# jermp/sshash

Hardware: AMD Instinct MI355X
Metric: k-mer Lookups/sec (batched random queries, bit-exact ids) (higher is better)
Workload: dtype u64

## Files before the change

### sshash_amd/csrc/engine.hip

```cpp
#include <hip/hip_runtime.h>

#include <algorithm>
#include <atomic>
#include <cstdlib>
#include <cstring>
#include <mutex>
#include <exception>
#include <stdexcept>
#include <thread>

#include "engine.hpp"
#include "hooks.hpp"
#include "replica.hpp"
#include "sktable.hpp"

namespace sshash_amd {

static void check_single_launch(uint64_t lanes, char const* what) {
    if (lanes >= (uint64_t(1) << 32))
        throw error(error_kind::argument, std::string(what) + ": at most 2^32 - 1 lanes per call (split the batch)");
}


int visible_device_count() {
// ... 103 lines not shown
        for (uint32_t b = a + 1; b < count;) {
            if (((e[a] >> 40) & 0xFFFF) == ((e[b] >> 40) & 0xFFFF)) {
                e[b] = e[count - 1];
                e[count - 1] = 0;
                --count;
                overflow = true;
            } else {
                ++b;
            }
        }
    }
    if (overflow) e[0] |= uint64_t(1) << 63;
    for (uint32_t j = 0; j < DIR_SLOTS; ++j) B[j] = e[j];
    if (overflow) atomicAdd(stats, 1ull);
    atomicAdd(stats + 1, (unsigned long long)count);
}

engine::engine(std::shared_ptr<host_index> idx) : m_idx(std::move(idx)) {}
engine::~engine() = default;

bool engine::on_device(int device) const {
    std::shared_lock<std::shared_mutex> lock(m_replicas_mutex);
    for (auto const& r : m_replicas)
        if (r->device == device) return true;
    return false;
}

std::vector<int> engine::devices() const {
    std::vector<int> d;
    std::shared_lock<std::shared_mutex> lock(m_replicas_mutex);
    for (auto const& r : m_replicas) d.push_back(r->device);
    return d;
}

uint64_t engine::device_bytes(int device) const { return replica(device)->bytes; }

void engine::device_stats(int device, uint64_t out[16]) const {
    device_replica const* r = replica(device);
    out[0] = r->bytes;
    out[1] = r->view.directory.enabled ? r->view.directory.num_buckets : 0;
    out[2] = r->directory_overflowed;
    out[3] = r->directory_entries;
    out[4] = r->view.sk.enabled ? uint64_t(r->view.sk.num_buckets) * SK_BUCKET_SLOTS +
                                      uint64_t(r->view.sk.kmer_buckets) * (r->view.k > 31 ? SK_BUCKET_SLOTS : SK_KMER_ENTRIES_NARROW)
                                : 0;
    out[5] = r->sk_keys;
    out[6] = r->sk_keys - r->sk_heavy_keys;
    out[7] = r->sk_unplaced;
    out[8] = r->sk_slots_used;
    out[9] = r->sk_heavy_keys;
    out[10] = r->sk_heavy_kmers;
    out[11] = r->view.sk.enabled ? 0 : r->sk_absent_reason;
    out[12] = r->sk_bytes;
    out[13] = r->view.sk.m;
    out[14] = out[15] = 0;
}

void engine::device_table_histogram(int device, uint64_t out[32]) const {
    device_replica const* r = replica(device);
    for (int i = 0; i < 32; ++i) out[i] = i < 20 && r->view.sk.enabled ? r->sk_histogram[i] : 0;
}

device_replica const* engine::replica(int device) const {
    std::shared_lock<std::shared_mutex> lock(m_replicas_mutex);
    for (auto const& r : m_replicas)
        if (r->device == device) return r.get();
    throw error(error_kind::no_device, "dictionary is not resident on device " + std::to_string(device) +
                             " (call sshash_to_device first)");
}

char const* isa_guard_state() {
#if defined(SSHASH_ISA_GUARDED)
    return "guarded";
#else
    return "plain";
#endif
}

void engine::to_device(int device, uint32_t table_shards, uint32_t table_shard_id) {
#if !defined(SSHASH_ISA_GUARDED)
    {
        static std::once_flag once;
        std::call_once(once, [] {
            fprintf(stderr, "[sshash_amd] WARNING: this library was NOT built through tools/isa_guard.py (make -C sshash_amd/csrc): on gfx950 a "
                                "kernel that keeps a 64-bit shift amount in the last VGPR of its allocation computes wrongly some of the time "
                                "(HISTORY.md); tests/test_isa_guard.py names the kernels of a build that are exposed\n");
        });
    }
#endif
    if (table_shards == 0 || table_shard_id >= table_shards) throw error(error_kind::argument, "table shard id must be < number of table shards");
    std::lock_guard<std::mutex> one_upload_at_a_time(m_upload_mutex);
    {
        std::shared_lock<std::shared_mutex> lock(m_replicas_mutex);
        for (auto const& r : m_replicas) {
            if (r->device != device) continue;
            if (r->view.sk.num_shards != table_shards || r->view.sk.shard_id != table_shard_id)
                throw error(error_kind::argument, "the dictionary is already resident on device " + std::to_string(device) +
                                                      " with another table sharding (" + std::to_string(r->view.sk.shard_id) + " of " +
                                                      std::to_string(r->view.sk.num_shards) + ")");
            return;
        }
    }
    const int count = visible_device_count();
    if (count == 0) throw error(error_kind::no_device, "no HIP device visible: the lookup path requires an MI355X (no CPU fallback)");
    if (device < 0 || device >= count) throw error(error_kind::no_device, "invalid device ordinal " + std::to_string(device));
    device_guard guard(device);
    host_index const& idx = *m_idx;
    auto rep = std::make_unique<device_replica>();
    rep->device = device;
    dict_view& v = rep->view;
    v.k = idx.k;
    v.m = idx.m;
    v.canonical = idx.canonical;
    v.skew_parts = idx.skew_num_partitions;
    v.hash_magic = idx.hash_magic;
    v.num_kmers = idx.num_kmers;
    v.num_strings = idx.num_strings;
    v.num_bases = idx.num_bases;
    {
        const uint32_t nt = std::max(1u, std::min(16u, std::thread::hardware_concurrency()));
        std::vector<granule> g = make_granules(idx, nt);
        if (idx.k <= 31) {
            std::vector<atom32> a = make_atoms(g, nt);
            std::vector<granule>().swap(g);
            v.granules = rep->put(a);
        } else {
            v.granules = rep->put(g);
        }
    }
    v.endpoints = rep->put(idx.endpoints);
    v.minimizers = rep->put_mphf(idx.minimizers_mphf);
    v.cw_width = idx.control_codewords.width;
    v.off_width = idx.mid_load_buckets.width;
    v.begin_buckets_of_size = rep->put(idx.begin_buckets_of_size);
    v.mid_load = rep->put(idx.mid_load_buckets.words);
    v.heavy_load = rep->put(idx.heavy_load_buckets.words);
    v.heavy_size = idx.heavy_load_buckets.size;
    v.codewords = nullptr;
    v.cw_packed = 0;
    v.directory.buckets = nullptr;
    v.directory.num_buckets = 0;
    v.directory.enabled = 0;
    rep->bytes_still_to_come = 8 * sizeof(skew_part_dev);
    for (uint32_t p = 0; p < 8; ++p) {
        if (p < idx.skew_num_partitions && idx.skew_mphfs[p].num_keys) {
            mphf_host const& f = idx.skew_mphfs[p];
            rep->bytes_still_to_come += f.parts.size() * sizeof(f.parts[0]) + (f.pilots.size() + f.free_slots.size() + idx.skew_positions[p].words.size()) * 8;
        } else {
            rep->bytes_still_to_come += 64;
        }
    }
    if (idx.weighted()) rep->bytes_still_to_come += (idx.weight_starts.size() + idx.weight_values.size()) * 8;
    build_sk_table(*rep, idx, table_shards, table_shard_id);
    const char* dir_env = std::getenv("SSHASH_AMD_DIRECTORY");
    const bool lean = v.sk.enabled && !(dir_env && dir_env[0] == '1');
    if (lean) {
        v.codewords = rep->put(idx.control_codewords.words);
        v.cw_packed = 1;
    } else {
        const uint64_t n = idx.control_codewords.size;
        device_buffers tmp;
        uint64_t* packed = tmp.alloc<uint64_t>(idx.control_codewords.words.size());
        HIP_CHECK(hipMemcpy(packed, idx.control_codewords.words.data(), idx.control_codewords.words.size() * sizeof(uint64_t), hipMemcpyHostToDevice));
        uint64_t* wide = tmp.alloc<uint64_t>(std::max<uint64_t>(n, 1));
        tmp.keep(wide, *rep);
        rep->bytes += std::max<uint64_t>(n, 1) * sizeof(uint64_t);
        if (n) {
            check_single_launch(n, "upload (one lane per minimizer)");
            hipLaunchKernelGGL(widen_codewords_kernel, dim3(uint32_t((n + 255) / 256)), dim3(256), 0, 0, v, packed, n, wide);
            HIP_CHECK(hipGetLastError());
            HIP_CHECK(hipDeviceSynchronize());
        }
        v.codewords = wide;
    }
    if (!lean) {
        const bool want = !(dir_env && dir_env[0] == '0');
        const uint64_t n = idx.control_codewords.size;
        const uint64_t nb = uint64_t(double(n) / DIR_LOAD) + 1;
        if (want && n && nb < (uint64_t(1) << 32) && v.cw_width <= DIR_CODE_BITS) {
            device_buffers tmp;
            uint64_t* buckets = tmp.alloc<uint64_t>(nb * 4);
            uint32_t* claimed = tmp.alloc<uint32_t>(nb);
            unsigned long long* stats = tmp.alloc<unsigned long long>(2);
            HIP_CHECK(hipMemset(buckets, 0, nb * 32));
            HIP_CHECK(hipMemset(claimed, 0, nb * 4));
            HIP_CHECK(hipMemset(stats, 0, 16));
            tmp.keep(buckets, *rep);
            rep->bytes += nb * 32;
            hipLaunchKernelGGL(directory_insert_kernel, dim3(uint32_t((n + 255) / 256)), dim3(256), 0, 0, v, n, buckets, claimed, uint32_t(nb));
            hipLaunchKernelGGL(directory_finalize_kernel, dim3(uint32_t((nb + 255) / 256)), dim3(256), 0, 0, buckets, claimed, uint32_t(nb), stats);
            HIP_CHECK(hipGetLastError());
            unsigned long long h_stats[2];
            HIP_CHECK(hipMemcpy(h_stats, stats, 16, hipMemcpyDeviceToHost));
            rep->directory_overflowed = h_stats[0];
            rep->directory_entries = h_stats[1];
            v.directory.buckets = buckets;
            v.directory.num_buckets = uint32_t(nb);
            v.directory.enabled = 1;
        }
    }
    std::vector<skew_part_dev> skew(8);
    for (uint32_t p = 0; p < 8; ++p) {
        std::memset(&skew[p], 0, sizeof(skew_part_dev));
        if (p < idx.skew_num_partitions && idx.skew_mphfs[p].num_keys) {
            skew[p].f = rep->put_mphf(idx.skew_mphfs[p]);
            skew[p].positions = rep->put(idx.skew_positions[p].words);
            skew[p].pos_width = idx.skew_positions[p].width;
        } else {
            mphf_host dummy;
            dummy.pilot_width = 1;
            dummy.num_keys = 1;
            mphf_partition part{};
            part.num_keys = 1;
            part.table_size = 1;
            part.dense_buckets = 1;
            part.sparse_buckets = 1;
            dummy.parts.push_back(part);
            dummy.pilots.assign(2, 0);
            dummy.free_slots.assign(1, 0);
            skew[p].f = rep->put_mphf(dummy);
            skew[p].positions = rep->put(std::vector<uint64_t>(2, 0));
            skew[p].pos_width = 1;
        }
    }
    rep->d_skew = rep->put(skew);
    v.weight_starts = v.weight_values = nullptr;
    v.num_weight_intervals = idx.weight_values.size();
    if (idx.weighted()) {
        v.weight_starts = rep->put(idx.weight_starts);
        v.weight_values = rep->put(idx.weight_values);
    }
    rep->create_scratch_pool();
    if (const uint64_t budget = hbm_budget(); budget && rep->bytes > budget)
        throw error(error_kind::no_device, "the replica needs " + std::to_string(rep->bytes) + " bytes of HBM, SSHASH_AMD_HBM_BUDGET allows " +
                                               std::to_string(budget) + ": partition the dictionary (minimizer shards, table shards)");
    std::unique_lock<std::shared_mutex> lock(m_replicas_mutex);
    m_replicas.push_back(std::move(rep));
}


template <int W, bool CANON, int MODE, bool ASCII>
__global__ void __launch_bounds__(256)
lookup_kernel(const dict_view d, const skew_part_dev* __restrict__ skew, const void* __restrict__ queries,
              const uint64_t n, const bool check_rc, const result_view out, uint8_t* __restrict__ member,
              const uint8_t* __restrict__ lane_valid) {
    const uint64_t stride = uint64_t(gridDim.x) * blockDim.x;
    for (uint64_t i = uint64_t(blockIdx.x) * blockDim.x + threadIdx.x; i < n; i += stride) {
        if (lane_valid && !(lane_valid[i] & 1)) continue;
        kmer_w<W> x;
        if constexpr (ASCII) {
            x = kmer_from_ascii<W>(static_cast<const char*>(queries) + i * d.k, d.k);
        } else {
            const uint64_t* q = static_cast<const uint64_t*>(queries) + i * W;
            for (int j = 0; j < W; ++j) x.w[j] = q[j];
            x = kmer_take_chars<W>(x, d.k);
        }
        const hit_t h = lookup_one<W, CANON, MODE != int(out_mode::full)>(d, skew, x, check_rc);
        if constexpr (MODE == int(out_mode::member)) {
            member[i] = h.found ? 1 : 0;
        } else {
            store_result<MODE == int(out_mode::full)>(d, out, i, h);
        }
    }
}

constexpr uint32_t DEFER_SHARDS = 2048;
constexpr uint32_t DEFER_BLOCKS_PER_SHARD = 4;

struct pass_queues {
    uint32_t* defer_counts;
    uint32_t* resume_counts;
    uint32_t* defer_index;
    uint32_t* resume_index;
    uint64_t* resume_kmers;
    uint64_t* resume_meta;
    uint32_t defer_capacity;
    uint32_t resume_capacity;
    uint32_t flag_misses;
};
constexpr uint32_t DEFER_FLAG_ONLY = 1u << 31;

template <int W, bool ASCII>
__device__ __forceinline__ kmer_w<W> load_query(const void* __restrict__ queries, uint64_t i, uint32_t k) {
    kmer_w<W> x;
    if constexpr (ASCII) {
        x = kmer_from_ascii<W>(static_cast<const char*>(queries) + i * k, k);
    } else {
        const uint64_t* q = static_cast<const uint64_t*>(queries) + i * W;
        for (int j = 0; j < W; ++j) x.w[j] = __builtin_nontemporal_load(q + j);
        x = kmer_take_chars<W>(x, k);
    }
    return x;
}

template <int W, bool CANON, int MODE, bool ASCII, bool SK>
__global__ void __launch_bounds__(256, (W == 2 && SK) ? 8 : 1)
fast_lookup_kernel(const dict_view d, const void* __restrict__ queries, const uint64_t n, const bool check_rc,
                   const result_view out, uint8_t* __restrict__ member, const pass_queues q,
                   const uint8_t* __restrict__ lane_valid ) {
    constexpr uint32_t TILE_WORDS = ASCII ? 64 * (W == 1 ? 31 : 63) + 24 : 0;
    constexpr uint32_t STAGE_WORDS = SK ? 256 * 16 : 0;
    __shared__ uint4 lds[(TILE_WORDS > STAGE_WORDS ? TILE_WORDS : STAGE_WORDS) / 4 + 1];
    const uint64_t i = uint64_t(blockIdx.x) * blockDim.x + threadIdx.x;
    const bool active = i < n && (!lane_valid || (lane_valid[i] & 1));
    kmer_w<W> x = kmer_zero<W>();
    if constexpr (ASCII) {
        uint32_t* tile = reinterpret_cast<uint32_t*>(lds);
        const uint64_t first = uint64_t(blockIdx.x) * blockDim.x;
        const uint32_t count = uint32_t(n - first < blockDim.x ? n - first : blockDim.x);
        const uint32_t bytes = count * d.k;
        const char* src = static_cast<const char*>(queries) + first * d.k;
        if ((reinterpret_cast<uintptr_t>(src) & 15) == 0) {
            for (uint32_t c = threadIdx.x; c * 16 < bytes; c += blockDim.x) {
                if (c * 16 + 16 <= bytes) {
                    reinterpret_cast<uint4*>(tile)[c] = sk_load_piece(src + 16 * c);
                } else {
                    for (uint32_t b = c * 16; b < bytes; ++b) reinterpret_cast<char*>(tile)[b] = src[b];
                }
            }
        } else {
            for (uint32_t b = threadIdx.x; b < bytes; b += blockDim.x) reinterpret_cast<char*>(tile)[b] = src[b];
        }
        __syncthreads();
        if (active) {
            const uint32_t start = threadIdx.x * d.k, w0 = start >> 2, sh = start & 3;
            uint32_t acc[2 * W];
#pragma unroll
            for (int t = 0; t < 2 * W; ++t) {
                acc[t] = 0;
                if (16u * uint32_t(t) < d.k) {
                    uint32_t prev = tile[w0 + 4 * t];
#pragma unroll
                    for (int j = 0; j < 4; ++j) {
                        const uint32_t next = tile[w0 + 4 * t + j + 1];
                        const uint32_t four = __builtin_amdgcn_alignbyte(next, prev, sh);
                        prev = next;
                        const uint32_t c = (((four >> 1) & 0x03030303u) * 0x01041040u) >> 24;
                        acc[t] |= c << (8 * j);
                    }
                }
            }
            x.w[0] = uint64_t(acc[0]) | (uint64_t(acc[1]) << 32);
            if constexpr (W == 2) x.w[1] = uint64_t(acc[2]) | (uint64_t(acc[3]) << 32);
            x = kmer_take_chars<W>(x, d.k);
        }
        if constexpr (SK) __syncthreads();
    } else {
        if (active) x = load_query<W, false>(queries, i, d.k);
    }
    fast_t r;
    const uint32_t shard = blockIdx.x & (DEFER_SHARDS - 1);
    if constexpr (SK) {
        if constexpr (W == 1)
            r = sk_lookup_in_wave<W>(d, x, active, CANON || check_rc, (!CANON && check_rc) ? int8_t(-1) : int8_t(1), lds + (threadIdx.x >> 6) * (64 * 4));
        else
            r = sk_first_pass_wave<W>(d, x, active, CANON || check_rc, (!CANON && check_rc) ? int8_t(-1) : int8_t(1),
                                      lds + (threadIdx.x >> 6) * (64 * 4));
        bool resume = active && r.outcome == FAST_CONTINUE;
        const uint32_t place = wave_queue_place(resume, q.resume_counts + shard);
        if (resume) {
            if (place < q.resume_capacity) {
                const uint64_t at = uint64_t(shard) * q.resume_capacity + place;
                q.resume_index[at] = uint32_t(i) | uint32_t(r.kmer_offset);
                for (int j = 0; j < W; ++j) q.resume_kmers[at * W + j] = x.w[j];
            } else {
                r.outcome = FAST_DEFER;
            }
        }
        if (!active) return;
    } else {
        bool by_pairs = false;
        if constexpr (W == 1 && !CANON) by_pairs = (d.num_bases >> 37) == 0;
        if (by_pairs) {
            if constexpr (W == 1 && !CANON) r = fast_lookup_pairs(d, x, active, check_rc);
        } else {
            r = active ? fast_lookup_one<W, CANON>(d, x, check_rc) : fast_unsettled(false);
        }
        const bool scan = active && r.outcome == FAST_SCAN;
        const uint32_t place = wave_queue_place(scan, q.resume_counts + shard);
        if (scan) {
            if (place < q.resume_capacity) {
                const uint64_t at = uint64_t(shard) * q.resume_capacity + place;
                q.resume_index[at] = uint32_t(i);
                q.resume_meta[at] = r.kmer_offset;
                for (int j = 0; j < W; ++j) q.resume_kmers[at * W + j] = x.w[j];
            } else {
                r.outcome = FAST_DEFER;
            }
        }
        if (!active) return;
    }
    if constexpr (MODE == int(out_mode::member)) {
        __builtin_nontemporal_store(uint8_t(r.outcome == FAST_HIT ? 1 : 0), member + i);
    } else {
        hit_t h;
        h.kmer_offset = r.kmer_offset;
        h.string_id = r.string_id;
        h.orientation = r.orientation;
        h.found = r.outcome == FAST_HIT;
        h.minimizer_found = true;
        store_result<MODE == int(out_mode::full)>(d, out, i, h);
    }
    if (r.outcome == FAST_DEFER) q.defer_index[uint64_t(shard) * q.defer_capacity + atomicAdd(q.defer_counts + shard, 1u)] = uint32_t(i);
    else if (MODE == int(out_mode::full) && SK && q.flag_misses && r.outcome == FAST_MISS)
        q.defer_index[uint64_t(shard) * q.defer_capacity + atomicAdd(q.defer_counts + shard, 1u)] = uint32_t(i) | DEFER_FLAG_ONLY;
}

constexpr uint32_t RESUME_PARTS = 4;

template <int W, bool CANON, int MODE>
__global__ void __launch_bounds__(256)
resume_lookup_kernel(const dict_view d, const bool check_rc, const result_view out, uint8_t* __restrict__ member, const pass_queues q) {
    __shared__ uint4 lds[256 * 4];
    const uint32_t shard = blockIdx.x & (DEFER_SHARDS - 1), part = blockIdx.x / DEFER_SHARDS;
    const uint32_t pushed = q.resume_counts[shard];
    const uint32_t total = pushed < q.resume_capacity ? pushed : q.resume_capacity;
    for (uint32_t base = part * blockDim.x; base < total; base += RESUME_PARTS * blockDim.x) {
        const uint32_t j = base + threadIdx.x;
        const bool active = j < total;
        const uint64_t at = uint64_t(shard) * q.resume_capacity + (active ? j : 0u);
        const uint32_t entry = q.resume_index[at];
        const uint64_t i = entry & ((1u << RESUME_CHOICE_SHIFT) - 1);
        kmer_w<W> x;
        for (int t = 0; t < W; ++t) x.w[t] = q.resume_kmers[at * W + t];
        const fast_t r = sk_second_pass_wave<W>(d, x, active, entry, CANON || check_rc, (!CANON && check_rc) ? int8_t(-1) : int8_t(1),
                                                lds + (threadIdx.x >> 6) * (64 * 4));
        if (!active) continue;
        if (r.outcome == FAST_DEFER) {
            q.defer_index[uint64_t(shard) * q.defer_capacity + atomicAdd(q.defer_counts + shard, 1u)] = uint32_t(i);
        } else if constexpr (MODE == int(out_mode::member)) {
            member[i] = r.outcome == FAST_HIT ? 1 : 0;
        } else {
            hit_t h;
            h.kmer_offset = r.kmer_offset;
            h.string_id = r.string_id;
            h.orientation = r.orientation;
            h.found = r.outcome == FAST_HIT;
            h.minimizer_found = true;
            store_result<MODE == int(out_mode::full)>(d, out, i, h);
            if (MODE == int(out_mode::full) && q.flag_misses && r.outcome == FAST_MISS)
                q.defer_index[uint64_t(shard) * q.defer_capacity + atomicAdd(q.defer_counts + shard, 1u)] = uint32_t(i) | DEFER_FLAG_ONLY;
        }
    }
}

template <int W, bool CANON, int MODE>
__global__ void __launch_bounds__(256)
scan_lookup_kernel(const dict_view d, const bool check_rc, const result_view out, uint8_t* __restrict__ member, const pass_queues q) {
    struct entry_t {
        uint64_t kmer[W];
        uint64_t meta;
        uint64_t offset;
        uint32_t string_id;
        uint32_t incl;
        int32_t orientation;
        uint32_t pad;
    };
    __shared__ entry_t lds[256];
    entry_t* E = lds + (threadIdx.x & ~63u);
    const uint32_t lane = threadIdx.x & 63u;
    const uint32_t shard = blockIdx.x & (DEFER_SHARDS - 1), part = blockIdx.x / DEFER_SHARDS;
    const uint32_t pushed = q.resume_counts[shard];
    const uint32_t total = pushed < q.resume_capacity ? pushed : q.resume_capacity;
    for (uint32_t base = part * blockDim.x; base < total; base += RESUME_PARTS * blockDim.x) {
        const uint32_t j = base + threadIdx.x;
        const bool active = j < total;
        const uint64_t at = uint64_t(shard) * q.resume_capacity + (active ? j : 0u);
        const uint32_t i = q.resume_index[at];
        const uint64_t meta = active ? q.resume_meta[at] : 0;
        const bool rc_strand = (meta >> 44) & 1;
        kmer_w<W> x;
        for (int t = 0; t < W; ++t) x.w[t] = q.resume_kmers[at * W + t];
        const kmer_w<W> y = (!CANON && rc_strand) ? kmer_revcomp<W>(x, d.k) : x;
        const uint32_t mine = active ? uint32_t((meta >> 32) & 63u) : 0u;
        uint32_t incl = mine;
        for (int o = 1; o < 64; o <<= 1) {
            const uint32_t up = __shfl_up(incl, o, 64);
            if (int(lane) >= o) incl += up;
        }
        for (int t = 0; t < W; ++t) E[lane].kmer[t] = y.w[t];
        E[lane].meta = meta;
        E[lane].offset = INVALID_U64;
        E[lane].string_id = 0;
        E[lane].incl = incl;
        E[lane].orientation = 1;
        const uint32_t all = __shfl(incl, 63, 64);
        __builtin_amdgcn_fence(__ATOMIC_RELEASE, "wavefront");
        __builtin_amdgcn_wave_barrier();
        __builtin_amdgcn_fence(__ATOMIC_ACQUIRE, "wavefront");
        for (uint32_t c0 = 0; c0 < all; c0 += 64) {
            const uint32_t t = c0 + lane;
            if (t < all) {
                uint32_t lo = 0, hi = 63;
                while (lo < hi) {
                    const uint32_t mid = (lo + hi) >> 1;
                    if (E[mid].incl > t) hi = mid;
                    else lo = mid + 1;
                }
                const uint64_t em = E[lo].meta;
                const uint32_t left = uint32_t((em >> 32) & 63u), pos = uint32_t((em >> 38) & 63u);
                const uint32_t c = t - (E[lo].incl - left) + 1;
                const uint64_t p = packed_get(d.mid_load, (em & 0xFFFFFFFFull) + c, d.off_width);
                kmer_w<W> want;
                for (int w = 0; w < W; ++w) want.w[w] = E[lo].kmer[w];
                if constexpr (CANON) {
                    const kmer_w<W> want_rc = kmer_revcomp<W>(want, d.k);
                    const uint32_t pos2 = d.k - d.m - pos;
                    const window_t<W> w1 = read_window<W>(d.granules, p >= pos ? p - pos : p, d.k);
                    const window_t<W> w2 = read_window<W>(d.granules, p >= pos2 ? p - pos2 : p, d.k);
                    const bool f1 = kmer_eq<W>(w1.kmer, want), b1 = kmer_eq<W>(w1.kmer, want_rc);
                    const bool f2 = kmer_eq<W>(w2.kmer, want), b2 = kmer_eq<W>(w2.kmer, want_rc);
                    if (p >= pos && (f1 || b1) && !w1.crosses) {
                        E[lo].offset = p - pos;
                        E[lo].string_id = w1.string_id;
                        E[lo].orientation = b1 ? -1 : 1;
                    } else if (p >= pos2 && (f2 || b2) && !w2.crosses) {
                        E[lo].offset = p - pos2;
                        E[lo].string_id = w2.string_id;
                        E[lo].orientation = b2 ? -1 : 1;
                    }
                } else {
                    if (p >= pos) {
                        const window_t<W> w = read_window<W>(d.granules, p - pos, d.k);
                        if (kmer_eq<W>(w.kmer, want) && !w.crosses) {
                            E[lo].offset = p - pos;
                            E[lo].string_id = w.string_id;
                        }
                    }
                }
            }
        }
        __builtin_amdgcn_fence(__ATOMIC_RELEASE, "wavefront");
        __builtin_amdgcn_wave_barrier();
        __builtin_amdgcn_fence(__ATOMIC_ACQUIRE, "wavefront");
        if (active) {
            hit_t h;
            h.kmer_offset = E[lane].offset;
            h.string_id = E[lane].string_id;
            h.found = h.kmer_offset != INVALID_U64;
            h.minimizer_found = true;
            h.orientation = CANON ? int8_t(E[lane].orientation) : (rc_strand ? int8_t(-1) : int8_t(1));
            if (!h.found && !CANON && !rc_strand && check_rc) {
                q.defer_index[uint64_t(shard) * q.defer_capacity + atomicAdd(q.defer_counts + shard, 1u)] = i;
            } else if constexpr (MODE == int(out_mode::member)) {
                member[i] = h.found ? 1 : 0;
            } else {
                store_result<MODE == int(out_mode::full)>(d, out, i, h);
            }
        }
        __builtin_amdgcn_wave_barrier();
    }
}

template <int W, bool CANON, int MODE, bool ASCII>
__global__ void __launch_bounds__(256)
deferred_lookup_kernel(const dict_view d, const skew_part_dev* __restrict__ skew, const void* __restrict__ queries,
                       const bool check_rc, const result_view out, uint8_t* __restrict__ member, const pass_queues q) {
    const uint32_t shard = blockIdx.x & (DEFER_SHARDS - 1), part = blockIdx.x / DEFER_SHARDS;
    const uint32_t total = q.defer_counts[shard];
    const uint32_t* mine = q.defer_index + uint64_t(shard) * q.defer_capacity;
    for (uint32_t j = part * blockDim.x + threadIdx.x; j < total; j += DEFER_BLOCKS_PER_SHARD * blockDim.x) {
        const uint32_t entry = mine[j];
        const uint64_t i = entry & ~DEFER_FLAG_ONLY;
        const kmer_w<W> x = load_query<W, ASCII>(queries, i, d.k);
        if constexpr (MODE == int(out_mode::full)) {
            if (q.flag_misses) {
                if (entry & DEFER_FLAG_ONLY) {
                    out.minimizer_found[i] = minimizer_found_of_a_miss<W, CANON>(d, skew, x, check_rc) ? 1 : 0;
                } else {
                    store_result<true>(d, out, i, lookup_one<W, CANON, false>(d, skew, x, check_rc));
                }
                continue;
            }
        }
        const hit_t h = lookup_one<W, CANON, true>(d, skew, x, check_rc);
        if constexpr (MODE == int(out_mode::member)) {
            member[i] = h.found ? 1 : 0;
        } else {
            store_result<MODE == int(out_mode::full)>(d, out, i, h);
        }
    }
}

static uint64_t launch_piece_queries() { return test_hook_u64("piece", uint64_t(1) << 27, 4096, uint64_t(1) << 27); }

static uint32_t resume_capacity_divisor() { return uint32_t(test_hook_u64("resume_divisor", 2, 1, 4096)); }

template <int W, bool CANON, int MODE, bool ASCII>
static void launch(device_replica const* rep, void const* q, uint64_t n, bool check_rc,
                   result_view const& out, uint8_t* member, hipStream_t stream, uint8_t const* lane_valid) {
    dict_view const& d = rep->view;
    skew_part_dev const* skew = rep->d_skew;
    const uint32_t block = 256;
    {
        const bool wants_flag = MODE == int(out_mode::full) && out.minimizer_found;
        if (!(wants_flag && !d.sk.enabled)) {
            const uint64_t piece_max = launch_piece_queries();
            uint64_t pieces = (n + piece_max - 1) / piece_max;
            const bool in_wave = W == 1 && d.sk.enabled;
            const uint64_t piece = ((n + pieces - 1) / pieces + block - 1) / block * block;
            pieces = (n + piece - 1) / piece;
            const bool overlap = pieces > 1 && in_wave;
            const size_t qbytes = size_t(W) * 8, kbytes = d.k;
            const uint32_t nblocks_max = uint32_t((std::min(piece, n) + block - 1) / block);
            pass_queues shape{};
            shape.defer_capacity = ((nblocks_max + DEFER_SHARDS - 1) / DEFER_SHARDS) * block;
            shape.resume_capacity = (shape.defer_capacity + 1) / resume_capacity_divisor();
            const uint64_t defer_places = uint64_t(DEFER_SHARDS) * shape.defer_capacity, resume_places = uint64_t(DEFER_SHARDS) * shape.resume_capacity;
            const size_t set_bytes =
                (2 * DEFER_SHARDS * sizeof(uint32_t) + (defer_places + resume_places) * sizeof(uint32_t) + resume_places * (W + 1) * sizeof(uint64_t) + 255) & ~size_t(255);
            std::lock_guard<std::mutex> enqueue(rep->launch_mutex);
            device_replica::stream_scratch& sc = rep->scratch_for(stream, (overlap ? 2 : 1) * set_bytes, overlap);
            uint64_t index = 0;
            for (uint64_t at = 0; at < n; at += piece, ++index) {
                const uint64_t m = std::min(piece, n - at);
                const uint32_t nblocks = uint32_t((m + block - 1) / block);
                const uint32_t set = overlap ? uint32_t(index & 1) : 0u;
                pass_queues pq = shape;
                pq.flag_misses = wants_flag ? 1u : 0u;
                char* scratch = static_cast<char*>(sc.block) + set * set_bytes;
                if (overlap && index >= 2) HIP_CHECK(hipStreamWaitEvent(stream, sc.tail_done[set], 0));
                HIP_CHECK(hipMemsetAsync(scratch, 0, 2 * DEFER_SHARDS * sizeof(uint32_t), stream));
                pq.defer_counts = reinterpret_cast<uint32_t*>(scratch);
                pq.resume_counts = pq.defer_counts + DEFER_SHARDS;
                pq.resume_kmers = reinterpret_cast<uint64_t*>(pq.resume_counts + DEFER_SHARDS);
                pq.resume_meta = pq.resume_kmers + resume_places * W;
                pq.defer_index = reinterpret_cast<uint32_t*>(pq.resume_meta + resume_places);
                pq.resume_index = pq.defer_index + defer_places;
                const void* qa = static_cast<const char*>(q) + at * (ASCII ? kbytes : qbytes);
                const result_view ids = advance(out, at);
                uint8_t* mem = member ? member + at : nullptr;
                hipStream_t tail = stream;
                if (d.sk.enabled) {
                    hipLaunchKernelGGL((fast_lookup_kernel<W, CANON, MODE, ASCII, true>), dim3(nblocks), dim3(block), 0, stream, d, qa,
                                       m, check_rc, ids, mem, pq, lane_valid ? lane_valid + at : nullptr);
                } else {
                    hipLaunchKernelGGL((fast_lookup_kernel<W, CANON, MODE, ASCII, false>), dim3(nblocks), dim3(block), 0, stream, d, qa,
                                       m, check_rc, ids, mem, pq, lane_valid ? lane_valid + at : nullptr);
                }
                if (overlap) {
                    HIP_CHECK(hipEventRecord(sc.first_done[set], stream));
                    HIP_CHECK(hipStreamWaitEvent(sc.aux, sc.first_done[set], 0));
                    tail = sc.aux;
                }
                if constexpr (W == 2) {
                    if (d.sk.enabled)
                        hipLaunchKernelGGL((resume_lookup_kernel<W, CANON, MODE>), dim3(DEFER_SHARDS * RESUME_PARTS), dim3(block), 0, tail, d,
                                           check_rc, ids, mem, pq);
                }
                if (!d.sk.enabled)
                    hipLaunchKernelGGL((scan_lookup_kernel<W, CANON, MODE>), dim3(DEFER_SHARDS * RESUME_PARTS), dim3(block), 0, tail, d,
                                       check_rc, ids, mem, pq);
                hipLaunchKernelGGL((deferred_lookup_kernel<W, CANON, MODE, ASCII>), dim3(DEFER_SHARDS * DEFER_BLOCKS_PER_SHARD), dim3(block), 0, tail, d,
                                   skew, qa, check_rc, ids, mem, pq);
                if (overlap) HIP_CHECK(hipEventRecord(sc.tail_done[set], sc.aux));
                HIP_CHECK(hipGetLastError());
            }
            if (overlap) HIP_CHECK(hipStreamWaitEvent(stream, sc.tail_done[(index - 1) & 1], 0));
            return;
        }
    }
    uint64_t blocks = (n + block - 1) / block;
    if (blocks > (uint64_t(1) << 22)) blocks = uint64_t(1) << 22;
    hipLaunchKernelGGL((lookup_kernel<W, CANON, MODE, ASCII>), dim3(uint32_t(blocks)), dim3(block), 0, stream, d, skew,
                       q, n, check_rc, out, member, lane_valid);
    HIP_CHECK(hipGetLastError());
}

template <int W, bool CANON, bool ASCII>
static void launch_mode(out_mode mode, device_replica const* rep, void const* q, uint64_t n,
                        bool check_rc, result_view const& out, uint8_t* member, hipStream_t s, uint8_t const* lane_valid) {
    switch (mode) {
        case out_mode::ids: launch<W, CANON, 0, ASCII>(rep, q, n, check_rc, out, member, s, lane_valid); break;
        case out_mode::full: launch<W, CANON, 1, ASCII>(rep, q, n, check_rc, out, member, s, lane_valid); break;
        case out_mode::member: launch<W, CANON, 2, ASCII>(rep, q, n, check_rc, out, member, s, lane_valid); break;
    }
}

template <bool ASCII>
static void launch_any(out_mode mode, device_replica const* rep, void const* q, uint64_t n,
                       bool check_rc, result_view const& out, uint8_t* member, hipStream_t s, uint8_t const* lane_valid = nullptr) {
    dict_view const& d = rep->view;
    const bool wide = d.k > 31;
    if (!wide && !d.canonical) launch_mode<1, false, ASCII>(mode, rep, q, n, check_rc, out, member, s, lane_valid);
    else if (!wide && d.canonical) launch_mode<1, true, ASCII>(mode, rep, q, n, check_rc, out, member, s, lane_valid);
    else if (wide && !d.canonical) launch_mode<2, false, ASCII>(mode, rep, q, n, check_rc, out, member, s, lane_valid);
    else launch_mode<2, true, ASCII>(mode, rep, q, n, check_rc, out, member, s, lane_valid);
}


static void check_outputs(out_mode mode, result_view const& out, uint8_t* member) {
    if (mode == out_mode::member) {
        if (!member) throw error(error_kind::argument, "is_member output pointer is null");
    } else if (!out.kmer_id) {
        throw error(error_kind::argument, "kmer_id output pointer is null");
    }
}

void engine::lookup_packed_masked_device(int device, uint64_t const* d_kmers, uint8_t const* d_lane_valid, uint64_t n, bool check_rc,
                                         out_mode mode, result_view const& d_out, void* stream) const {
    device_replica const* rep = replica(device);
    check_outputs(mode, d_out, nullptr);
    if (n == 0) return;
    device_guard guard(device);
    launch_any<false>(mode, rep, d_kmers, n, check_rc, d_out, nullptr, hipStream_t(stream), d_lane_valid);
}

void engine::lookup_packed_device(int device, uint64_t const* d_kmers, uint64_t n, bool check_rc, out_mode mode,
                                  result_view const& d_out, uint8_t* d_member, void* stream) const {
    device_replica const* rep = replica(device);
    check_outputs(mode, d_out, d_member);
    if (n == 0) return;
    device_guard guard(device);
    launch_any<false>(mode, rep, d_kmers, n, check_rc, d_out, d_member, hipStream_t(stream));
}

void engine::lookup_ascii_device(int device, char const* d_kmers, uint64_t n, bool check_rc, out_mode mode,
                                 result_view const& d_out, uint8_t* d_member, void* stream) const {
    device_replica const* rep = replica(device);
    check_outputs(mode, d_out, d_member);
    if (n == 0) return;
    device_guard guard(device);
    launch_any<true>(mode, rep, d_kmers, n, check_rc, d_out, d_member, hipStream_t(stream));
}


template <int W>
__global__ void __launch_bounds__(256)
expand_neighbours_kernel(const uint64_t* __restrict__ kmers, const uint64_t n, const uint32_t k, uint64_t* __restrict__ out) {
    const uint64_t t = uint64_t(blockIdx.x) * blockDim.x + threadIdx.x;
    if (t >= 8 * n) return;
    const kmer_w<W> x = load_query<W, false>(kmers, t >> 3, k);
    const kmer_w<W> y = kmer_neighbour<W>(x, uint32_t(t & 7), k);
    for (int j = 0; j < W; ++j) out[t * W + j] = y.w[j];
}

void engine::neighbours_packed_device(int device, uint64_t const* d_kmers, uint64_t n, bool check_rc, out_mode mode,
                                      result_view const& d_out, void* stream) const {
    device_replica const* rep = replica(device);
    check_outputs(mode, d_out, nullptr);
    if (n == 0) return;
    device_guard guard(device);
    hipStream_t s = hipStream_t(stream);
    const uint32_t W = rep->view.k <= 31 ? 1 : 2;
    check_single_launch(8 * n, "kmer_neighbours");
    device_buffers tmp(rep, s);
    uint64_t* expanded = tmp.alloc<uint64_t>(8 * n * W);
    const dim3 grid(uint32_t((8 * n + 255) / 256)), block(256);
    if (W == 1) hipLaunchKernelGGL(expand_neighbours_kernel<1>, grid, block, 0, s, d_kmers, n, rep->view.k, expanded);
    else hipLaunchKernelGGL(expand_neighbours_kernel<2>, grid, block, 0, s, d_kmers, n, rep->view.k, expanded);
    HIP_CHECK(hipGetLastError());
    launch_any<false>(mode, rep, expanded, 8 * n, check_rc, d_out, nullptr, s);
}

void engine::neighbours_packed_host(uint64_t const* h_kmers, uint64_t n, bool check_rc, out_mode mode,
                                    result_view const& h_out) const {
    const uint32_t k = m_idx->k, W = m_idx->words_per_kmer();
    std::vector<uint64_t> expanded(8 * n * W);
    for (uint64_t i = 0; i < n; ++i) {
        for (uint32_t which = 0; which < 8; ++which) {
            if (W == 1) {
                kmer_w<1> x;
                x.w[0] = h_kmers[i];
                expanded[8 * i + which] = kmer_neighbour<1>(kmer_take_chars<1>(x, k), which, k).w[0];
            } else {
                kmer_w<2> x;
                x.w[0] = h_kmers[2 * i];
                x.w[1] = h_kmers[2 * i + 1];
                const kmer_w<2> y = kmer_neighbour<2>(kmer_take_chars<2>(x, k), which, k);
                expanded[2 * (8 * i + which)] = y.w[0];
                expanded[2 * (8 * i + which) + 1] = y.w[1];
            }
        }
    }
    lookup_packed_host(expanded.data(), 8 * n, check_rc, mode, h_out, nullptr);
}

void engine::string_neighbours_host(uint64_t const* h_string_ids, uint64_t n, bool check_rc, out_mode mode,
                                    result_view const& h_out) const {
    host_index const& idx = *m_idx;
    const uint32_t k = idx.k, W = idx.words_per_kmer();
    std::vector<uint64_t> expanded(8 * n * W);
    uint64_t first[2], last[2];
    for (uint64_t i = 0; i < n; ++i) {
        const uint64_t s = h_string_ids[i];
        if (s >= idx.num_strings) throw error(error_kind::argument, "string_id out of range");
// ... 654 lines not shown
```

### sshash_amd/csrc/hooks.hpp

```cpp
#pragma once

#include <cstdint>
#include <cstdlib>
#include <cstring>
#include <memory>
#include <mutex>
#include <string>

namespace sshash_amd {

struct hook_snapshot {
    std::mutex m;
    std::shared_ptr<const std::string> text;
};
inline hook_snapshot& hook_state() {
    static hook_snapshot s;
    return s;
}
inline void test_hooks_refresh() {
    char const* e = std::getenv("SSHASH_AMD_TEST_HOOKS");
    hook_snapshot& st = hook_state();
    std::lock_guard<std::mutex> lock(st.m);
    if (!e || !*e) st.text.reset();
    else if (!st.text || *st.text != e) st.text = std::make_shared<const std::string>(e);
}

inline std::string test_hook_value(char const* name, bool& found) {
    found = false;
    std::shared_ptr<const std::string> text;
    {
        hook_snapshot& st = hook_state();
        std::lock_guard<std::mutex> lock(st.m);
        text = st.text;
    }
    if (!text) return {};
    const size_t n = std::strlen(name);
    for (char const* p = text->c_str(); *p;) {
        if (std::strncmp(p, name, n) == 0 && p[n] == '=') {
            char const* v = p + n + 1;
            char const* end = std::strchr(v, ',');
            found = true;
            return end ? std::string(v, end) : std::string(v);
        }
        p = std::strchr(p, ',');
        if (!p) break;
        ++p;
    }
    return {};
}

inline uint64_t test_hook_u64(char const* name, uint64_t fallback, uint64_t lo, uint64_t hi) {
    bool found;
    const std::string t = test_hook_value(name, found);
    if (!found) return fallback;
    const uint64_t v = std::strtoull(t.c_str(), nullptr, 10);
    return v >= lo && v <= hi ? v : fallback;
}

inline double test_hook_f64(char const* name, double fallback, double lo, double hi) {
    bool found;
    const std::string t = test_hook_value(name, found);
    if (!found) return fallback;
    const double v = std::strtod(t.c_str(), nullptr);
    return v >= lo && v <= hi ? v : fallback;
}

}
```

### sshash_amd/csrc/lookup_device.hpp

```cpp
#pragma once

#include <hip/hip_runtime.h>

#include "device_layout.hpp"

namespace sshash_amd {

struct skew_part_dev {
    mphf_view f;
    uint64_t const* positions;
    uint32_t pos_width;
    uint32_t pad;
};

struct hit_t {
    uint64_t kmer_offset;
    uint32_t string_id;
    int8_t orientation;
    bool found;
    bool minimizer_found;
};

template <int W>
struct window_t {
// ... 749 lines not shown
};

__device__ __forceinline__ sk_walk_t sk_walk_begin(sk_hash_t const& h, uint32_t c) {
    sk_walk_t w;
    w.h = h;
    w.c = c;
    w.back_to = SK_NO_RETURN;
    w.on_kmer_sequence = false;
    return w;
}

template <int W>
__device__ __forceinline__ void sk_walk_to_kmer_sequence(dict_view const& d, kmer_w<W> const& x, kmer_w<W> const& x_rc, sk_walk_t& w,
                                                         sk_query_t<W>& Q, bool go_on) {
    w.back_to = go_on ? w.c + 1 : SK_NO_RETURN;
    w.h = sk_hash_kmer_region(sk_kmer_key<W>(x, x_rc), d.sk.num_buckets, d.sk.kmer_buckets);
    w.c = 0;
    w.on_kmer_sequence = true;
    Q.fingerprint = w.h.fingerprint;
}

template <int W>
__device__ __forceinline__ bool sk_walk_step(dict_view const& d, kmer_w<W> const& x, kmer_w<W> const& x_rc, sk_key_t const& kk,
                                             sk_walk_t& w, sk_query_t<W>& Q, fast_t& r, uint32_t go_on, bool marker) {
    if (r.outcome != FAST_MISS) return false;
    if (marker && !w.on_kmer_sequence) {
        sk_walk_to_kmer_sequence<W>(d, x, x_rc, w, Q, go_on != 0);
        return true;
    }
    if (go_on != 0) {
        if (++w.c < SK_CHOICES) return true;
        r.outcome = FAST_DEFER;
        return false;
    }
    if (w.on_kmer_sequence && w.back_to != SK_NO_RETURN) {
        w.c = w.back_to;
        w.back_to = SK_NO_RETURN;
        if (w.c >= SK_CHOICES) {
            r.outcome = FAST_DEFER;
            return false;
        }
        w.h = sk_hash(kk.key, d.sk.num_buckets);
        Q.fingerprint = w.h.fingerprint;
        return true;
    }
    return false;
}


template <int OWNER>
__device__ __forceinline__ uint32_t quad_broadcast(uint32_t v) {
    return uint32_t(__builtin_amdgcn_mov_dpp(int(v), OWNER * 0x55, 0xf, 0xf, true));
}


__device__ __forceinline__ void sk_wave_sync() {
    asm volatile("s_waitcnt vmcnt(0) lgkmcnt(0)" ::: "memory");
    __builtin_amdgcn_wave_barrier();
    asm volatile("" ::: "memory");
}

template <int W, bool MIXED = false>
__device__ __forceinline__ void sk_stage_lines(dict_view const& d, uint32_t bucket, uint32_t line, bool need, uint4* wave_stage, bool kmer_region = false) {
    char const* slots = static_cast<char const*>(d.sk.slots);
    const uint32_t sub = threadIdx.x & 3u;
    const uint32_t mine = need ? bucket : 0u, my_line = need ? line : 0u;
    const uint32_t b0 = quad_broadcast<0>(mine), b1 = quad_broadcast<1>(mine), b2 = quad_broadcast<2>(mine), b3 = quad_broadcast<3>(mine);
    uint32_t l0 = 0, l1 = 0, l2 = 0, l3 = 0;
    if constexpr (W == 2) {
        l0 = quad_broadcast<0>(my_line);
        l1 = quad_broadcast<1>(my_line);
        l2 = quad_broadcast<2>(my_line);
        l3 = quad_broadcast<3>(my_line);
    }
    uint64_t a0 = uint64_t(b0) * (64 * W) + 64 * l0, a1 = uint64_t(b1) * (64 * W) + 64 * l1, a2 = uint64_t(b2) * (64 * W) + 64 * l2,
             a3 = uint64_t(b3) * (64 * W) + 64 * l3;
    if constexpr (W == 2 && MIXED) {
        const uint32_t mine_region = need && kmer_region ? 1u : 0u;
        const uint64_t base = uint64_t(d.sk.num_buckets) * 128, first = d.sk.num_buckets;
        if (quad_broadcast<0>(mine_region)) a0 = base + uint64_t(b0 - first) * 64;
        if (quad_broadcast<1>(mine_region)) a1 = base + uint64_t(b1 - first) * 64;
        if (quad_broadcast<2>(mine_region)) a2 = base + uint64_t(b2 - first) * 64;
        if (quad_broadcast<3>(mine_region)) a3 = base + uint64_t(b3 - first) * 64;
    }
    const uint32_t lane = threadIdx.x & 63u;
    const uint4 p0 = sk_load_piece(slots + a0 + 16 * sub), p1 = sk_load_piece(slots + a1 + 16 * sub),
                p2 = sk_load_piece(slots + a2 + 16 * sub), p3 = sk_load_piece(slots + a3 + 16 * sub);
    wave_stage[0 * 64 + lane] = p0;
    wave_stage[1 * 64 + lane] = p1;
    wave_stage[2 * 64 + lane] = p2;
    wave_stage[3 * 64 + lane] = p3;
    __builtin_amdgcn_fence(__ATOMIC_RELEASE, "wavefront");
    __builtin_amdgcn_wave_barrier();
    __builtin_amdgcn_fence(__ATOMIC_ACQUIRE, "wavefront");
}

template <int W, bool MIXED = false>
__device__ __forceinline__ void sk_probe_bucket_wave(dict_view const& d, sk_query_t<W> const& Q, uint32_t bucket, uint32_t c, bool need,
                                                     uint4* wave_stage, fast_t& r, bool& key_seen, bool& marker, uint32_t& go_on,
                                                     bool kmer_region = false) {
    const uint32_t lane = threadIdx.x & 63u;
    const uint4* mine = wave_stage + (lane & 3u) * 64 + (lane >> 2) * 4;
    sk_bucket_flags flags;
    flags.go_on = 0;
    flags.second_used = false;
    sk_stage_lines<W, MIXED>(d, bucket, 0u, need, wave_stage, kmer_region);
    bool compact = false;
    if constexpr (MIXED) compact = kmer_region;
    if (need && !compact) {
        sk_examine_slot<W, true>(d, Q, c, [mine](uint32_t i) { return mine[i]; }, r, key_seen, marker, flags);
        if constexpr (W == 1) sk_examine_slot<W, false>(d, Q, c, [mine](uint32_t i) { return mine[2 + i]; }, r, key_seen, marker, flags);
    }
    if constexpr (W == 2 && MIXED) {
        if (need && compact) {
            sk_examine_kmer_entry<true>(Q, c, [mine](uint32_t i) { return mine[i]; }, r, flags);
            sk_examine_kmer_entry<false>(Q, c, [mine](uint32_t i) { return mine[2 + i]; }, r, flags);
        }
    }
    if constexpr (W == 1 && MIXED) {
        if (need && compact) {
            const uint32_t* words = reinterpret_cast<const uint32_t*>(mine);
            sk_examine_kmer_line(Q, c, [words](uint32_t i) { return words[i]; }, r, flags);
        }
    }
    if constexpr (W == 2) {
        bool second = need && r.outcome == FAST_MISS && flags.second_used;
        uint32_t* posted = reinterpret_cast<uint32_t*>(wave_stage + 64);
        char const* slots = static_cast<char const*>(d.sk.slots);
#pragma unroll 1
        for (;;) {
            sk_wave_sync();
            const uint64_t mask = __ballot(second);
            if (mask == 0) break;
            const uint32_t rank = uint32_t(__popcll(mask & ((uint64_t(1) << lane) - 1)));
            const bool served = second && rank < 16;
            if (lane < 16) posted[lane] = 0u;
            sk_wave_sync();
            if (served) posted[rank] = bucket;
            sk_wave_sync();
            const uint32_t b = posted[lane >> 2];
            wave_stage[lane] = sk_load_piece(slots + uint64_t(b) * 128 + 64 + 16 * (lane & 3u));
            sk_wave_sync();
            if (served) {
                const uint4* line = wave_stage + 4 * rank;
                sk_examine_slot<W, false>(d, Q, c, [line](uint32_t i) { return line[i]; }, r, key_seen, marker, flags);
                second = false;
            }
        }
    }
    go_on = flags.go_on;
    __builtin_amdgcn_wave_barrier();
}

constexpr uint32_t RESUME_CHOICE_SHIFT = 27;
constexpr uint32_t RESUME_HEAVY = 1u << 30;
constexpr uint32_t RESUME_GO_ON = 1u << 31;

template <int W>
__device__ __forceinline__ fast_t sk_first_pass_wave(dict_view const& d, kmer_w<W> const& x, bool active, bool allow_rc,
                                                     int8_t miss_orientation, uint4* wave_stage) {
    const kmer_w<W> x_rc = kmer_revcomp<W>(x, d.k);
    const sk_key_t kk = sk_key<W>(x, x_rc, d.k, d.sk.m);
    const bool usable = active && sk_usable(d, kk);
    const sk_hash_t h = sk_hash(kk.key, d.sk.num_buckets);
    const sk_query_t<W> Q = sk_make_query<W>(x, x_rc, kk, h.fingerprint);
    fast_t r = fast_unsettled(active && !usable);
    uint32_t go_on = 0;
    bool marker = false, key_seen = false;
    sk_probe_bucket_wave<W>(d, Q, usable ? h.bucket[0] : 0u, 0u, usable, wave_stage, r, key_seen, marker, go_on);
    if constexpr (W == 2) {
        bool hop = usable && r.outcome == FAST_MISS && marker;
        if (__ballot(hop) != 0) {
            const sk_hash_t hk = sk_hash_kmer_region(sk_kmer_key<W>(x, x_rc), d.sk.num_buckets, d.sk.kmer_buckets);
            sk_query_t<W> Qk = Q;
            Qk.fingerprint = hk.fingerprint;
            const uint32_t lane = threadIdx.x & 63u;
            uint32_t* posted = reinterpret_cast<uint32_t*>(wave_stage + 64);
            char const* slots = static_cast<char const*>(d.sk.slots);
            uint32_t kmer_go_on = 0;
            bool pending = hop;
#pragma unroll 1
            for (;;) {
                sk_wave_sync();
                const uint64_t mask = __ballot(pending);
                if (mask == 0) break;
                const uint32_t rank = uint32_t(__popcll(mask & ((uint64_t(1) << lane) - 1)));
                const bool served = pending && rank < 16;
                if (lane < 16) posted[lane] = 0u;
                sk_wave_sync();
                if (served) posted[rank] = 2 * d.sk.num_buckets + (hk.bucket[0] - d.sk.num_buckets);
                sk_wave_sync();
                const uint32_t line = posted[lane >> 2];
                wave_stage[lane] = sk_load_piece(slots + uint64_t(line) * 64 + 16 * (lane & 3u));
                sk_wave_sync();
                if (served) {
                    const uint4* mine = wave_stage + 4 * rank;
                    sk_bucket_flags flags;
                    sk_examine_kmer_entry<true>(Qk, 0u, [mine](uint32_t i) { return mine[i]; }, r, flags);
                    sk_examine_kmer_entry<false>(Qk, 0u, [mine](uint32_t i) { return mine[2 + i]; }, r, flags);
                    kmer_go_on = flags.go_on;
                    pending = false;
                }
            }
            if (hop && r.outcome == FAST_MISS && kmer_go_on == 0) {
                marker = false;
            }
        }
    }
    if (usable) {
        if (r.outcome == FAST_MISS) {
            if (marker) {
                r.outcome = FAST_CONTINUE;
                r.kmer_offset = RESUME_HEAVY | (go_on ? RESUME_GO_ON : 0u);
            } else if (go_on) {
                r.outcome = FAST_CONTINUE;
                r.kmer_offset = 1u << RESUME_CHOICE_SHIFT;
            } else {
                r.orientation = miss_orientation;
            }
        } else if (r.orientation < 0 && !allow_rc) {
            r = fast_unsettled(false);
            r.orientation = miss_orientation;
        }
    }
    return r;
}

__device__ __forceinline__ void sk_finish_in_wave(dict_view const& d, kmer_w<1> const& x, kmer_w<1> const& x_rc, sk_key_t const& kk, sk_walk_t& w,
                                                  sk_query_t<1>& Q, fast_t& r, bool need, uint4* wave_stage) {
    const uint32_t lane = threadIdx.x & 63u;
    char const* slots = static_cast<char const*>(d.sk.slots);
    uint32_t* posted = reinterpret_cast<uint32_t*>(wave_stage + 64);
#pragma unroll 1
    for (;;) {
        const uint64_t mask = __ballot(need);
        if (mask == 0) break;
        const uint32_t rank = uint32_t(__popcll(mask & ((uint64_t(1) << lane) - 1)));
        const bool served = need && rank < 16;
        if (lane < 16) posted[lane] = 0u;
        sk_wave_sync();
        if (served) posted[rank] = sk_choice(w.h, w.c);
        sk_wave_sync();
        const uint32_t b = posted[lane >> 2];
        wave_stage[lane] = sk_load_piece(slots + uint64_t(b) * 64 + 16 * (lane & 3u));
        sk_wave_sync();
        if (served) {
            const uint4* mine = wave_stage + 4 * rank;
            sk_bucket_flags flags;
            flags.go_on = 0;
            flags.second_used = false;
            bool marker = false, key_seen = false;
            if (sk_choice(w.h, w.c) >= d.sk.num_buckets) {
                const uint32_t* words = reinterpret_cast<const uint32_t*>(mine);
                sk_examine_kmer_line(Q, w.c, [words](uint32_t i) { return words[i]; }, r, flags);
            } else {
                sk_examine_slot<1, true>(d, Q, w.c, [mine](uint32_t i) { return mine[i]; }, r, key_seen, marker, flags);
                sk_examine_slot<1, false>(d, Q, w.c, [mine](uint32_t i) { return mine[2 + i]; }, r, key_seen, marker, flags);
            }
            const uint32_t go_on = flags.go_on;
            need = sk_walk_step<1>(d, x, x_rc, kk, w, Q, r, go_on, marker);
        }
        sk_wave_sync();
    }
}

template <int W>
__device__ __forceinline__ fast_t sk_lookup_in_wave(dict_view const& d, kmer_w<W> const& x, bool active, bool allow_rc, int8_t miss_orientation,
                                                    uint4* wave_stage) {
    const kmer_w<W> x_rc = kmer_revcomp<W>(x, d.k);
    const sk_key_t kk = sk_key<W>(x, x_rc, d.k, d.sk.m);
    const bool usable = active && sk_usable(d, kk);
    sk_walk_t w = sk_walk_begin(sk_hash(kk.key, d.sk.num_buckets), 0);
    sk_query_t<W> Q = sk_make_query<W>(x, x_rc, kk, w.h.fingerprint);
    fast_t r = fast_unsettled(active && !usable);
    uint32_t go_on = 0;
    bool marker = false, key_seen = false;
    sk_probe_bucket_wave<W>(d, Q, usable ? w.h.bucket[0] : 0u, 0u, usable, wave_stage, r, key_seen, marker, go_on);
    sk_wave_sync();
    bool need = false;
    if (usable) need = sk_walk_step<W>(d, x, x_rc, kk, w, Q, r, go_on, marker);
    sk_finish_in_wave(d, x, x_rc, kk, w, Q, r, need, wave_stage);
    if (usable && (r.outcome == FAST_MISS || (r.outcome == FAST_HIT && r.orientation < 0 && !allow_rc))) {
        r = fast_unsettled(false);
        r.orientation = miss_orientation;
    }
    return r;
}

template <int W>
__device__ __forceinline__ fast_t sk_second_pass_wave(dict_view const& d, kmer_w<W> const& x, bool active, uint32_t entry, bool allow_rc,
                                                      int8_t miss_orientation, uint4* wave_stage) {
    const kmer_w<W> x_rc = kmer_revcomp<W>(x, d.k);
    const sk_key_t kk = sk_key<W>(x, x_rc, d.k, d.sk.m);
    sk_walk_t w = sk_walk_begin(sk_hash(kk.key, d.sk.num_buckets), (entry >> RESUME_CHOICE_SHIFT) & 7u);
    sk_query_t<W> Q = sk_make_query<W>(x, x_rc, kk, w.h.fingerprint);
    if (entry & RESUME_HEAVY) sk_walk_to_kmer_sequence<W>(d, x, x_rc, w, Q, (entry & RESUME_GO_ON) != 0);
    fast_t r = fast_unsettled(false);
    bool need = active;
#pragma unroll 1
    while (__ballot(need) != 0) {
        uint32_t go_on = 0;
        bool marker = false, key_seen = false;
        const uint32_t bucket = need ? sk_choice(w.h, w.c) : 0u;
        sk_probe_bucket_wave<W, true>(d, Q, bucket, w.c, need, wave_stage, r, key_seen, marker, go_on, bucket >= d.sk.num_buckets);
        if (need) need = sk_walk_step<W>(d, x, x_rc, kk, w, Q, r, go_on, marker);
    }
    if (r.outcome == FAST_MISS || (r.outcome == FAST_HIT && r.orientation < 0 && !allow_rc)) {
        r = fast_unsettled(false);
        r.orientation = miss_orientation;
    }
    return r;
}

__device__ __forceinline__ uint32_t wave_queue_place(bool push, uint32_t* counter) {
    const uint64_t mask = __ballot(push);
    if (mask == 0) return 0;
    const uint32_t lane = threadIdx.x & 63u;
    const uint32_t leader = uint32_t(__ffsll((unsigned long long)mask)) - 1u;
    uint32_t base = 0;
    if (lane == leader) base = atomicAdd(counter, uint32_t(__popcll(mask)));
    base = __shfl(base, int(leader), 64);
    return base + uint32_t(__popcll(mask & ((uint64_t(1) << lane) - 1)));
}

template <bool FULL>
__device__ __forceinline__ void store_result(dict_view const& d, result_view const& out, uint64_t i, hit_t const& h) {
    __builtin_nontemporal_store(h.found ? h.kmer_offset - uint64_t(h.string_id) * (d.k - 1) : INVALID_U64, out.kmer_id + i);
    if constexpr (FULL) {
        uint64_t begin = INVALID_U64, end = INVALID_U64;
        if (h.found && (out.string_begin || out.string_end || out.kmer_id_in_string)) {
            begin = d.endpoints[h.string_id];
            end = d.endpoints[h.string_id + 1];
        }
        if (out.kmer_id_in_string) __builtin_nontemporal_store(h.found ? h.kmer_offset - begin : INVALID_U64, out.kmer_id_in_string + i);
        if (out.kmer_offset) __builtin_nontemporal_store(h.found ? h.kmer_offset : INVALID_U64, out.kmer_offset + i);
        if (out.string_id) __builtin_nontemporal_store(h.found ? uint64_t(h.string_id) : INVALID_U64, out.string_id + i);
        if (out.string_begin) __builtin_nontemporal_store(begin, out.string_begin + i);
        if (out.string_end) __builtin_nontemporal_store(end, out.string_end + i);
        if (out.kmer_orientation) __builtin_nontemporal_store(h.orientation, out.kmer_orientation + i);
        if (out.minimizer_found) __builtin_nontemporal_store(uint8_t(h.minimizer_found ? 1 : 0), out.minimizer_found + i);
    }
}

}
```

Measured before the change: 38.11 billion.

## Fetch k=63 super-k-mer buckets with unit-stride cooperative loads through LDS

Adds a W==2 bucket-probe path in which each group of 8 lanes fetches one 128-byte bucket as 16-byte pieces. Four buckets per round are gathered via ds_bpermute of the lanes' bucket indices, and the pieces are staged into swizzled LDS so each owning lane can examine its slots. The intent is coalesced bucket reads instead of the previous per-wave probe pattern. It also pins the query k-mer in registers, recomputes x from the query at the end to reduce register pressure, and adds a bounds check that the slot allocation covers 128 bytes per bucket. The new path is enabled by default through a test hook.

Result: no change. 38.14 billion (median of 2 runs) (+0.1%).

```diff
diff --git a/sshash_amd/csrc/engine.hip b/sshash_amd/csrc/engine.hip
--- a/sshash_amd/csrc/engine.hip
+++ b/sshash_amd/csrc/engine.hip
@@ -279,6 +279,8 @@
     }
     if (idx.weighted()) rep->bytes_still_to_come += (idx.weight_starts.size() + idx.weight_values.size()) * 8;
     build_sk_table(*rep, idx, table_shards, table_shard_id);
+    if (rep->view.sk.enabled && idx.k > 31 && rep->sk_bytes < uint64_t(rep->view.sk.num_buckets) * 128)
+        throw error(error_kind::internal, "super-k-mer table: the keys' region ends beyond the allocation");
     const char* dir_env = std::getenv("SSHASH_AMD_DIRECTORY");
     const bool lean = v.sk.enabled && !(dir_env && dir_env[0] == '1');
     if (lean) {
@@ -420,7 +422,7 @@
     return x;
 }
 
-template <int W, bool CANON, int MODE, bool ASCII, bool SK>
+template <int W, bool CANON, int MODE, bool ASCII, bool SK, bool UNIT = false>
 __global__ void __launch_bounds__(256, (W == 2 && SK) ? 8 : 1)
 fast_lookup_kernel(const dict_view d, const void* __restrict__ queries, const uint64_t n, const bool check_rc,
                    const result_view out, uint8_t* __restrict__ member, const pass_queues q,
@@ -481,8 +483,8 @@
         if constexpr (W == 1)
             r = sk_lookup_in_wave<W>(d, x, active, CANON || check_rc, (!CANON && check_rc) ? int8_t(-1) : int8_t(1), lds + (threadIdx.x >> 6) * (64 * 4));
         else
-            r = sk_first_pass_wave<W>(d, x, active, CANON || check_rc, (!CANON && check_rc) ? int8_t(-1) : int8_t(1),
-                                      lds + (threadIdx.x >> 6) * (64 * 4));
+            r = sk_first_pass_wave<W, UNIT>(d, x, active, CANON || check_rc, (!CANON && check_rc) ? int8_t(-1) : int8_t(1),
+                                            lds + (threadIdx.x >> 6) * (64 * 4));
         bool resume = active && r.outcome == FAST_CONTINUE;
         const uint32_t place = wave_queue_place(resume, q.resume_counts + shard);
         if (resume) {
@@ -713,6 +715,8 @@
 
 static uint32_t resume_capacity_divisor() { return uint32_t(test_hook_u64("resume_divisor", 2, 1, 4096)); }
 
+static bool k63_unit_fetch() { return test_hook_u64("k63_unit_fetch", K63_UNIT_FETCH_DEFAULT, 0, 1) != 0; }
+
 template <int W, bool CANON, int MODE, bool ASCII>
 static void launch(device_replica const* rep, void const* q, uint64_t n, bool check_rc,
                    result_view const& out, uint8_t* member, hipStream_t stream, uint8_t const* lane_valid) {
@@ -725,6 +729,7 @@
             const uint64_t piece_max = launch_piece_queries();
             uint64_t pieces = (n + piece_max - 1) / piece_max;
             const bool in_wave = W == 1 && d.sk.enabled;
+            const bool unit_fetch = k63_unit_fetch();
             const uint64_t piece = ((n + pieces - 1) / pieces + block - 1) / block * block;
             pieces = (n + piece - 1) / piece;
             const bool overlap = pieces > 1 && in_wave;
@@ -758,7 +763,11 @@
                 const result_view ids = advance(out, at);
                 uint8_t* mem = member ? member + at : nullptr;
                 hipStream_t tail = stream;
-                if (d.sk.enabled) {
+                if (W == 2 && d.sk.enabled && unit_fetch) {
+                    if constexpr (W == 2)
+                        hipLaunchKernelGGL((fast_lookup_kernel<W, CANON, MODE, ASCII, true, true>), dim3(nblocks), dim3(block), 0, stream, d, qa,
+                                           m, check_rc, ids, mem, pq, lane_valid ? lane_valid + at : nullptr);
+                } else if (d.sk.enabled) {
                     hipLaunchKernelGGL((fast_lookup_kernel<W, CANON, MODE, ASCII, true>), dim3(nblocks), dim3(block), 0, stream, d, qa,
                                        m, check_rc, ids, mem, pq, lane_valid ? lane_valid + at : nullptr);
                 } else {
diff --git a/sshash_amd/csrc/hooks.hpp b/sshash_amd/csrc/hooks.hpp
--- a/sshash_amd/csrc/hooks.hpp
+++ b/sshash_amd/csrc/hooks.hpp
@@ -57,6 +57,8 @@
     return v >= lo && v <= hi ? v : fallback;
 }
 
+constexpr uint64_t K63_UNIT_FETCH_DEFAULT = 1;
+
 inline double test_hook_f64(char const* name, double fallback, double lo, double hi) {
     bool found;
     const std::string t = test_hook_value(name, found);
diff --git a/sshash_amd/csrc/lookup_device.hpp b/sshash_amd/csrc/lookup_device.hpp
--- a/sshash_amd/csrc/lookup_device.hpp
+++ b/sshash_amd/csrc/lookup_device.hpp
@@ -925,26 +925,71 @@
     __builtin_amdgcn_wave_barrier();
 }
 
+__device__ __forceinline__ void sk_probe_bucket_unit(dict_view const& d, sk_query_t<2> const& Q, uint32_t bucket, bool need, uint4* wave_stage,
+                                                     fast_t& r, bool& key_seen, bool& marker, uint32_t& go_on) {
+    const uint32_t lane = threadIdx.x & 63u;
+    const uint32_t group = lane >> 3, sub = lane & 7u;
+    char const* slots = static_cast<char const*>(d.sk.slots);
+    const uint32_t mine = need ? bucket : 0u;
+    const uint32_t put = 8 * group + (sub ^ group);
+    const uint32_t swizzle = lane & 7u;
+    const uint4* staged = wave_stage + 8 * (lane & 31u);
+    sk_bucket_flags flags;
+    flags.go_on = 0;
+    flags.second_used = false;
+#pragma unroll 1
+    for (uint32_t round = 0; round < 2; ++round) {
+        const uint32_t first = 32 * round + group;
+        const uint32_t b0 = uint32_t(__builtin_amdgcn_ds_bpermute(int(4 * first), int(mine))),
+                       b1 = uint32_t(__builtin_amdgcn_ds_bpermute(int(4 * (first + 8)), int(mine))),
+                       b2 = uint32_t(__builtin_amdgcn_ds_bpermute(int(4 * (first + 16)), int(mine))),
+                       b3 = uint32_t(__builtin_amdgcn_ds_bpermute(int(4 * (first + 24)), int(mine)));
+        const uint4 p0 = sk_load_piece(slots + uint64_t(b0) * 128 + 16 * sub), p1 = sk_load_piece(slots + uint64_t(b1) * 128 + 16 * sub),
+                    p2 = sk_load_piece(slots + uint64_t(b2) * 128 + 16 * sub), p3 = sk_load_piece(slots + uint64_t(b3) * 128 + 16 * sub);
+        __builtin_amdgcn_fence(__ATOMIC_RELEASE, "wavefront");
+        __builtin_amdgcn_wave_barrier();
+        wave_stage[0 * 64 + put] = p0;
+        wave_stage[1 * 64 + put] = p1;
+        wave_stage[2 * 64 + put] = p2;
+        wave_stage[3 * 64 + put] = p3;
+        __builtin_amdgcn_fence(__ATOMIC_RELEASE, "wavefront");
+        __builtin_amdgcn_wave_barrier();
+        __builtin_amdgcn_fence(__ATOMIC_ACQUIRE, "wavefront");
+        if (need && (lane >> 5) == round) {
+            sk_examine_slot<2, true>(d, Q, 0u, [staged, swizzle](uint32_t i) { return staged[i ^ swizzle]; }, r, key_seen, marker, flags);
+            if (r.outcome == FAST_MISS && flags.second_used)
+                sk_examine_slot<2, false>(d, Q, 0u, [staged, swizzle](uint32_t i) { return staged[(4 + i) ^ swizzle]; }, r, key_seen, marker, flags);
+        }
+    }
+    go_on = flags.go_on;
+    __builtin_amdgcn_wave_barrier();
+}
+
 constexpr uint32_t RESUME_CHOICE_SHIFT = 27;
 constexpr uint32_t RESUME_HEAVY = 1u << 30;
 constexpr uint32_t RESUME_GO_ON = 1u << 31;
 
-template <int W>
-__device__ __forceinline__ fast_t sk_first_pass_wave(dict_view const& d, kmer_w<W> const& x, bool active, bool allow_rc,
+template <int W, bool UNIT = false>
+__device__ __forceinline__ fast_t sk_first_pass_wave(dict_view const& d, kmer_w<W>& x, bool active, bool allow_rc,
                                                      int8_t miss_orientation, uint4* wave_stage) {
     const kmer_w<W> x_rc = kmer_revcomp<W>(x, d.k);
     const sk_key_t kk = sk_key<W>(x, x_rc, d.k, d.sk.m);
     const bool usable = active && sk_usable(d, kk);
     const sk_hash_t h = sk_hash(kk.key, d.sk.num_buckets);
-    const sk_query_t<W> Q = sk_make_query<W>(x, x_rc, kk, h.fingerprint);
+    sk_query_t<W> Q = sk_make_query<W>(x, x_rc, kk, h.fingerprint);
+    if constexpr (W == 2 && UNIT) {
+        for (int t = 0; t < W; ++t) asm volatile("" : "+v"(Q.y.w[t]), "+v"(Q.y_rc.w[t]));
+    }
     fast_t r = fast_unsettled(active && !usable);
     uint32_t go_on = 0;
     bool marker = false, key_seen = false;
-    sk_probe_bucket_wave<W>(d, Q, usable ? h.bucket[0] : 0u, 0u, usable, wave_stage, r, key_seen, marker, go_on);
+    if constexpr (W == 2 && UNIT) sk_probe_bucket_unit(d, Q, usable ? h.bucket[0] : 0u, usable, wave_stage, r, key_seen, marker, go_on);
+    else sk_probe_bucket_wave<W>(d, Q, usable ? h.bucket[0] : 0u, 0u, usable, wave_stage, r, key_seen, marker, go_on);
     if constexpr (W == 2) {
         bool hop = usable && r.outcome == FAST_MISS && marker;
         if (__ballot(hop) != 0) {
-            const sk_hash_t hk = sk_hash_kmer_region(sk_kmer_key<W>(x, x_rc), d.sk.num_buckets, d.sk.kmer_buckets);
+            const uint64_t kmer_key = (W == 2 && UNIT) ? sk_kmer_key<W>(Q.y, Q.y_rc) : sk_kmer_key<W>(x, x_rc);
+            const sk_hash_t hk = sk_hash_kmer_region(kmer_key, d.sk.num_buckets, d.sk.kmer_buckets);
             sk_query_t<W> Qk = Q;
             Qk.fingerprint = hk.fingerprint;
             const uint32_t lane = threadIdx.x & 63u;
@@ -996,6 +1041,7 @@
             r.orientation = miss_orientation;
         }
     }
+    if constexpr (W == 2 && UNIT) x = kmer_pick<W>(Q.s, Q.y_rc, Q.y);
     return r;
 }
 
```
